# holoskii/Rendering

Hardware: AMD Instinct MI355X
Metric: Mrays/s + ms/frame at 4096^2, 250k-tri BVH scene (higher is better)
Workload: dtype f32

## Files before the change

### include/rtx_debug.h

```cpp
#ifndef RTX_DEBUG_H
#define RTX_DEBUG_H
#include "rtx.h"
#ifdef __cplusplus
extern "C" {
#endif

int rtx_frame_mode(rtx_scene* scene, int* mode, float* split_ms, float* fused_ms);
int rtx_set_frame_mode(rtx_scene* scene, int mode);

int rtx_mesh_flatten_probe(const rtx_mesh* mesh, uint32_t* n_wide, void* wide_out, void* prune_out, uint32_t cap_wide, float* root_rec8);
int rtx_wide_node_slots(void);

int rtx_source_p_probe(const float* tris9, uint32_t n, const double* S3, double sigma, int cam, float* out);

int rtx_cost_grid_read(rtx_scene* scene, uint32_t* out, size_t n, uint32_t* grid_w, uint32_t* grid_h);

int rtx_set_knob(rtx_scene* scene, const char* name, double value);

#define RTX_VARIANT_BOXES    1u
#define RTX_VARIANT_PLAIN    2u
#define RTX_VARIANT_ANALYTIC 4u
#define RTX_VARIANT_STATS    8u
#define RTX_VARIANT_CULL     16u
int rtx_kernel_variant(rtx_scene* scene, uint32_t* bits);

int rtx_ssaa_list_read(rtx_scene* scene, uint32_t* info, uint32_t* scan, size_t n);

int rtx_kernel_time_reset(rtx_scene* scene);
int rtx_kernel_time_stats(rtx_scene* scene, int which, uint32_t* launches, double* total_ms);

int rtx_tile_cost_read(rtx_scene* scene, uint32_t* out, size_t n);

int rtx_math_probe(int device, int op, uint32_t n, const float* x, const float* y, float* out);

int rtx_vec_probe(int device, int op, uint32_t n, const float* a, const float* b, float ior, float* out);

int rtx_desc_serialize(const rtx_scene_desc* desc, void* out, size_t cap, size_t* need);

int rtx_bvh_build_mode(int mode);
int rtx_bvh_launches(const rtx_bvh* bvh, uint32_t* launches, int* queued);

int rtx_scene_mesh_read(rtx_scene* scene, uint32_t mesh, uint32_t* counts2, float* node_bounds, int32_t* node_skip, int32_t* leaf_begin,
                        int32_t* leaf_count, uint32_t* refs);
int rtx_scene_mesh_flat_read(rtx_scene* scene, uint32_t mesh, uint32_t* n_wide, void* wide_out, void* prune_out, uint32_t cap_wide, float* root_rec8);
int rtx_scene_edit_times(rtx_scene* scene, float* ms4);

int rtx_live_device_memory(size_t* allocations, size_t* bytes);

#ifdef __cplusplus
}
#endif
#endif
```

### rendering_amd/__init__.py

```python
import ctypes as C
import os

import numpy as np

HERE = os.path.dirname(os.path.abspath(__file__))
ROOT = os.path.dirname(HERE)
LIB_RTX = os.path.join(HERE, "librtx_hip.so")
LIB_HOST = os.path.join(HERE, "librendering_host.so")

__all__ = ["load", "Scene", "Comm", "RtxError", "device_count", "math_probe", "gather_plan", "exported_symbols"]


class RtxError(RuntimeError):
    pass


class Counters(C.Structure):
    _fields_ = [("rays", C.c_uint64), ("box_tests", C.c_uint64), ("tri_tests", C.c_uint64), ("moot_rays", C.c_uint64)]


_rtx = None
_host = None

RTX_SYMBOLS = [
    "rtx_last_error", "rtx_device_count", "rtx_scene_create", "rtx_scene_destroy", "rtx_scene_set_view", "rtx_scene_bytes",
    "rtx_render_pass1", "rtx_sobel", "rtx_render_ssaa", "rtx_render_frame", "rtx_render_ac", "rtx_frame_status", "rtx_frame_mode", "rtx_set_frame_mode", "rtx_set_knob", "rtx_cost_grid_read", "rtx_mesh_flatten_probe", "rtx_wide_node_slots", "rtx_source_p_probe", "rtx_quantize_bgr8", "rtx_render_frame_host",
    "rtx_counters_enable", "rtx_counters_reset", "rtx_counters_read", "rtx_last_kernel_ms", "rtx_math_probe",
    "rtx_cast_rays", "rtx_trace_rays", "rtx_kernel_time_reset", "rtx_kernel_time_stats", "rtx_tile_cost_read", "rtx_set_row_ownership",
    "rtx_bvh_build", "rtx_bvh_info", "rtx_bvh_read", "rtx_bvh_destroy",
    "rtx_vec_probe", "rtx_desc_serialize", "rtx_bvh_build_mode", "rtx_bvh_launches", "rtx_comm_unique_id", "rtx_comm_create", "rtx_comm_info", "rtx_comm_destroy", "rtx_comm_agree", "rtx_gather", "rtx_gather_plan",
    "rtx_scene_mesh_read", "rtx_scene_mesh_flat_read", "rtx_scene_edit_times", "rtx_kernel_variant", "rtx_ssaa_list_read", "rtx_live_device_memory",
]

RTX_EDIT_SYMBOLS = ["rtx_scene_set_object", "rtx_scene_update_mesh"]

RTX_QUERY_SYMBOLS = ["rtx_occluded_rays"]


def load():
    global _rtx, _host
    if _rtx is not None:
        return _rtx, _host
    for p in (LIB_RTX, LIB_HOST):
        if not os.path.exists(p):
            raise RtxError("native library %s is missing -- build it with ./build.sh (hipcc, gfx950); "
                           "there is no CPU fallback" % p)
    try:
        import torch
    except Exception:
        pass
    rtx = C.CDLL(LIB_RTX, mode=C.RTLD_GLOBAL)
    host = C.CDLL(LIB_HOST, mode=C.RTLD_GLOBAL)
    rtx.rtx_last_error.restype = C.c_char_p
    vp, u32, i32 = C.c_void_p, C.c_uint32, C.c_int
    rtx.rtx_device_count.argtypes = [C.POINTER(C.c_int)]
    rtx.rtx_render_pass1.argtypes = [vp, u32, u32, vp, vp]
    rtx.rtx_sobel.argtypes = [vp, vp, u32, u32, vp, vp]
    rtx.rtx_render_ssaa.argtypes = [vp, vp, u32, u32, vp, vp]
    rtx.rtx_render_frame.argtypes = [vp, u32, u32, vp, vp, vp]
    rtx.rtx_render_ac.argtypes = [vp, vp, vp, vp]
    rtx.rtx_frame_status.argtypes = [vp, C.POINTER(C.c_uint32)]
    rtx.rtx_set_frame_mode.argtypes = [vp, C.c_int]
    rtx.rtx_set_knob.argtypes = [vp, C.c_char_p, C.c_double]
    rtx.rtx_cost_grid_read.argtypes = [vp, vp, C.c_size_t, C.POINTER(C.c_uint32), C.POINTER(C.c_uint32)]
# ... 38 lines not shown
    host.rah_last_error.restype = C.c_char_p
    host.rah_scene_load.restype = vp
    host.rah_scene_load.argtypes = [C.c_char_p, C.c_char_p, i32, i32]
    host.rah_scene_free.argtypes = [vp]
    host.rah_scene_dims.argtypes = [vp] + [C.POINTER(C.c_int)] * 4
    host.rah_scene_resize.argtypes = [vp, i32, i32]
    host.rah_scene_set_device.argtypes = [vp, i32]
    host.rah_set_flag.argtypes = [vp, C.c_char_p, i32]
    host.rah_flatten.restype = vp
    host.rah_flatten.argtypes = [vp]
    host.rah_flat_desc.restype = vp
    host.rah_flat_desc.argtypes = [vp]
    host.rah_flat_free.argtypes = [vp]
    host.rah_bvh_counts.argtypes = [vp, i32, vp]
    host.rah_scene_gpu.restype = vp
    host.rah_scene_gpu.argtypes = [vp]
    host.rah_render_host.argtypes = [vp, vp, i32]
    host.rah_save_bmp.argtypes = [vp, vp, C.c_char_p]
    host.rah_bvh_dump.argtypes = [vp, i32, vp, vp, vp, vp, vp]
    host.rah_tris.argtypes = [vp, i32, vp]
    host.rah_camera.argtypes = [vp, vp, vp, vp, vp]
    host.rah_scene_digest.argtypes = [vp, vp, i32]
    host.rah_view_flags.argtypes = [vp]
    host.rah_load_bmp.argtypes = [C.c_char_p, C.POINTER(C.c_int), C.POINTER(C.c_int), vp, i32]
    host.rah_object_move.argtypes = [vp, i32] + [vp] * 5
    host.rah_object_type.argtypes = [vp, i32]
    host.rah_object_move_times.argtypes = [vp, vp]
    rtx.rtx_scene_set_object.argtypes = [vp, C.c_uint32, vp]
    rtx.rtx_scene_update_mesh.argtypes = [vp, C.c_uint32, vp, vp, vp, vp, vp, i32, vp]
    rtx.rtx_scene_mesh_read.argtypes = [vp, C.c_uint32] + [vp] * 6
    rtx.rtx_scene_mesh_flat_read.argtypes = [vp, C.c_uint32, vp, vp, vp, C.c_uint32, vp]
    rtx.rtx_scene_edit_times.argtypes = [vp, vp]
    rtx.rtx_kernel_variant.argtypes = [vp, C.POINTER(C.c_uint32)]
    rtx.rtx_ssaa_list_read.argtypes = [vp, vp, vp, C.c_size_t]
    rtx.rtx_live_device_memory.argtypes = [C.POINTER(C.c_size_t), C.POINTER(C.c_size_t)]
    _rtx, _host = rtx, host
    return rtx, host


def exported_symbols():
    rtx, _ = load()
    missing = [s for s in RTX_SYMBOLS + RTX_EDIT_SYMBOLS + RTX_QUERY_SYMBOLS if not hasattr(rtx, s)]
    return list(RTX_SYMBOLS), missing


VARIANT_BITS = {"boxes": 1, "plain": 2, "analytic": 4, "stats": 8, "cull": 16}


def _check(rc, what):
    if rc != 0:
        raise RtxError("%s failed (%d): %s" % (what, rc, _rtx.rtx_last_error().decode(errors="replace")))


def device_count():
    rtx, _ = load()
    n = C.c_int(0)
    _check(rtx.rtx_device_count(C.byref(n)), "rtx_device_count")
    return n.value


def live_device_memory():
    rtx, _ = load()
    n, b = C.c_size_t(0), C.c_size_t(0)
    _check(rtx.rtx_live_device_memory(C.byref(n), C.byref(b)), "rtx_live_device_memory")
    return n.value, b.value

# ... 270 lines not shown
                if torch.cuda.is_available():
                    return C.c_void_p(torch.cuda.current_stream().cuda_stream)
            except Exception:
                pass
            return None
        return C.c_void_p(getattr(stream, "cuda_stream", stream))

    def render_pass1(self, fb, rows=None, stream=None):
        r0, r1 = rows if rows is not None else (0, self.height)
        _check(self.rtx.rtx_render_pass1(self.gpu(), r0, r1, C.c_void_p(fb.data_ptr()), self._stream_ptr(stream)),
               "rtx_render_pass1")

    def sobel(self, fb, mask, rows=None, stream=None):
        r0, r1 = rows if rows is not None else (0, self.height)
        _check(self.rtx.rtx_sobel(self.gpu(), C.c_void_p(fb.data_ptr()), r0, r1, C.c_void_p(mask.data_ptr()),
                                  self._stream_ptr(stream)), "rtx_sobel")

    def render_ssaa(self, mask, fb, rows=None, stream=None):
        r0, r1 = rows if rows is not None else (0, self.height)
        _check(self.rtx.rtx_render_ssaa(self.gpu(), C.c_void_p(mask.data_ptr()), r0, r1, C.c_void_p(fb.data_ptr()),
                                        self._stream_ptr(stream)), "rtx_render_ssaa")

    def render_frame(self, fb, mask, rows=None, stream=None):
        r0, r1 = rows if rows is not None else (0, self.height)
        _check(self.rtx.rtx_render_frame(self.gpu(), r0, r1, C.c_void_p(fb.data_ptr()), C.c_void_p(mask.data_ptr()),
                                         self._stream_ptr(stream)), "rtx_render_frame")

    def render_ac(self, fb, counts=None, stream=None):
        cp = C.c_void_p(counts.data_ptr()) if counts is not None else None
        _check(self.rtx.rtx_render_ac(self.gpu(), C.c_void_p(fb.data_ptr()), cp, self._stream_ptr(stream)), "rtx_render_ac")

    def set_knob(self, name, value):
        _check(self.rtx.rtx_set_knob(self.gpu(), name.encode(), float(value)), "rtx_set_knob")

    def kernel_variant(self):
        b = C.c_uint32(0)
        _check(self.rtx.rtx_kernel_variant(self.gpu(), C.byref(b)), "rtx_kernel_variant")
        return {k: bool(b.value & bit) for k, bit in VARIANT_BITS.items()}

    def ssaa_list(self):
        g = self.gpu()
        info = np.zeros(16, np.uint32)
        _check(self.rtx.rtx_ssaa_list_read(g, _np_ptr(info), None, 0), "rtx_ssaa_list_read")
        d = dict(local=bool(info[0]), flagged=int(info[1]), sparse=bool(info[2]), tiles=int(info[3]), tiles_x=int(info[4]),
                 heavy_ticks=int(info[5]), spread_slots=int(info[6]), very=int(info[7]), spread_px=int(info[8]),
                 split4=int(info[9]), split16=int(info[10]), cost_sum=int(info[11]) | int(info[12]) << 32, frame_waves=int(info[13]), scan=None)
        if d["tiles"]:
            scan = np.zeros(2 * d["tiles"] + 1, np.uint32)
            _check(self.rtx.rtx_ssaa_list_read(g, _np_ptr(info), _np_ptr(scan), scan.size), "rtx_ssaa_list_read")
            d["scan"] = scan
        return d

    def cost_grid(self):
        gw, gh = C.c_uint32(0), C.c_uint32(0)
        _check(self.rtx.rtx_cost_grid_read(self.gpu(), None, 0, C.byref(gw), C.byref(gh)), "rtx_cost_grid_read")
        g = np.zeros((gh.value, gw.value, 2), np.uint32)
        _check(self.rtx.rtx_cost_grid_read(self.gpu(), _np_ptr(g), g.size, C.byref(gw), C.byref(gh)), "rtx_cost_grid_read")
        return g[..., 0], g[..., 1]

    def frame_status(self):
        st = C.c_uint32(0)
        _check(self.rtx.rtx_frame_status(self.gpu(), C.byref(st)), "rtx_frame_status")
        return st.value

    def set_frame_mode(self, mode):
        _check(self.rtx.rtx_set_frame_mode(self.gpu(), int(mode)), "rtx_set_frame_mode")
# ... 179 lines not shown
```

### rendering_amd/csrc/rtx_api.hip

```cpp
#include <hip/hip_runtime.h>

#include <cstdio>
#include <dlfcn.h>
#include <algorithm>
#include <array>
#include <functional>
#include <cmath>
#include <cstring>
#include <memory>
#include <string>
#include <type_traits>
#include <vector>

#include "../../include/rtx.h"
#include "../../include/rtx_debug.h"
#include "../../include/rtx_scene_edit.h"
#include "../../include/rtx_query.h"
#include "rtx_device.h"
#include "rtx_own.h"

using namespace rtxd;
using rtxown::DevArray; using rtxown::DevBag; using rtxown::Event; using rtxown::PinnedArray;

#include "rtx_kernels.hip"
#include "rtx_source.hip"
#include "rtx_rays.hip"

hipError_t rtxSortRayKeys(void* temp, size_t* tempBytes, const uint32_t* keysIn, uint32_t* keysOut, uint32_t* order, uint32_t n, int endBit,
                          hipStream_t st);

namespace {

thread_local std::string gErr;

struct RoctxApi { int (*push)(const char*) = nullptr; int (*pop)() = nullptr; };
const RoctxApi& roctx()
{
	static const RoctxApi api = [] {
		RoctxApi a;
		if (!getenv("ROCP_TOOL_LIBRARIES") && !getenv("RTX_ROCTX")) return a;
		void* h = dlopen("librocprofiler-sdk-roctx.so.1", RTLD_NOW | RTLD_GLOBAL);
		if (!h) h = dlopen("libroctx64.so.4", RTLD_NOW | RTLD_GLOBAL);
		if (!h) return a;
		a.push = (int (*)(const char*))dlsym(h, "roctxRangePushA");
		a.pop = (int (*)())dlsym(h, "roctxRangePop");
		if (!a.push || !a.pop) a = RoctxApi();
		return a;
	}();
	return api;
}
struct RoctxRange {
	bool on;
	explicit RoctxRange(const char* name) : on(roctx().push != nullptr) { if (on) roctx().push(name); }
	~RoctxRange() { if (on) roctx().pop(); }
};

int scanExclusive(uint32_t* data, uint32_t n, uint32_t* tmp, hipStream_t st, uint32_t& launches);

int fail(int code, const std::string& msg) { gErr = msg; return code; }
// ... 20 lines not shown
{
	const uint32_t t = m.refs[ref];
	const float* p = m.tri_pos + (size_t)t * 9;
	a.v0x = p[0]; a.v0y = p[1]; a.v0z = p[2]; a.tri = t;
	b.e1x = p[3] - p[0]; b.e1y = p[4] - p[1]; b.e1z = p[5] - p[2];
	b.e2x = p[6] - p[0]; c.e2y = p[7] - p[1]; c.e2z = p[8] - p[2];
}

}

struct Knobs {
	int pass1BlocksPerCU = 0, ssaaBlocksPerCU = 0, frameBlocksPerCU = 0;
	bool prune = true;
	bool sources = true;
	int pruneBoxes = -1;
	bool estimate = true;
	bool estimateShadows = true;
	float costPerRef = 2.0f, costPerLeaf = 95.0f, costBase = 6100.0f;
	float fatFactor = 3.0f;
	uint32_t stripLimit = 100000u;
	uint32_t heavyTicks = 18000u;
	uint32_t spreadSlots = 1u << 20;
	uint32_t splitPercent = 100;
	long long localBelow = -1;
	long long sparseBelow = -1;
	int frameMode = -1;
	uint32_t frameRuleTiles = 65536u, frameRuleTilesAnalytic = 8192u;
	uint32_t frameQueueCap = 0;
	bool debugItems = false;
	int traceReorder = -1;
	int traceOriginFirst = 1;
	int occludedSceneOrder = 0;
	uint32_t dbgTile = 0;
};

struct rtx_scene {
	int device = 0;
	int numCUs = 0;
	Knobs knobs;
	DevBag owned;
	std::vector<Mesh> meshRecs;
	std::vector<DevBag> meshOwned;
	std::vector<Object> objectRecs;
	std::vector<rtx_object> objectDescs;
	DevArray<float> sphereLeafDev;
	DevArray<char> flatScratch;
	float editMs[4] = { 0, 0, 0, 0 };
	Params params;
	bool stats = false;
	bool analytic = true;
	bool boxPrune = false;
	bool plain = true;
	DevArray<float> frames; size_t framesArea = 0;
	DevArray<uint32_t> tileCost, items; size_t tileCap = 0;
	DevArray<uint32_t> ssaaPixels;
	DevArray<uint32_t> work;
	DevArray<unsigned long long> counters;
	DevArray<uint32_t> orderWork;
	int blocksPass1 = 0, blocksSsaa = 0, blocksFrame = 0;
	DevArray<uint32_t> tileDeps; DevArray<unsigned long long> tileFlags; DevArray<uint8_t> tileClass;
	DevArray<unsigned long long> ssaaQueue;
	DevArray<unsigned long long> frameCtl;
	uint32_t epoch = 0;
	std::vector<float> meshBounds;
	struct TileQueues {
		std::vector<uint32_t> key;
		uint32_t* list = nullptr;
		uint8_t* need = nullptr; uint32_t listed = 0;
		uint32_t* countExpect = nullptr; bool needValid = false;
		bool costValid = false;
		uint64_t lastUse = 0;
		float frameMs[2] = { -1.f, -1.f };
		uint32_t frameSamples[2] = { 0, 0 };
		uint32_t framesSeen = 0, generation = 0;
		bool fusedGaveUp = false;
		hipStream_t builtOn = nullptr; Event builtEv;
		void forget()
		{
			key.clear(); costValid = false;
			frameMs[0] = frameMs[1] = -1.f; frameSamples[0] = frameSamples[1] = 0; framesSeen = 0; generation++; fusedGaveUp = false;
		}
	};
	struct LastFused { bool valid = false; uint32_t rowBegin = 0, rowEnd = 0; float* fb = nullptr; uint8_t* mask = nullptr; void* stream = nullptr; size_t queue = ~(size_t)0; uint32_t generation = 0;
	                   uint64_t viewSerial = 0; uint32_t bandH = 0, nParts = 0, part = 0, halo = 0; };
	LastFused lastFused;
	uint32_t framesRecovered = 0;
	DevArray<uint32_t> acCounts, acMax;
	DevArray<uint32_t> rayKeys, rayOrder; size_t rayCap = 0;
// ... 36 lines not shown
	size_t lastFrameQueue = ~(size_t)0;
	std::vector<TileQueues> tileQueues;
	uint64_t tileUse = 0;
	std::vector<Event> evPool[5];
	size_t evUsed[5] = { 0, 0, 0, 0, 0 };
	bool evCollect = false;
};

namespace {

void readKnobs(Knobs& k)
{
	const char* allow = ::getenv("RTX_ALLOW_ENV_KNOBS");
	if (!(allow && allow[0] == '1')) return;
	auto getenv = [](const char* name) { return ::getenv(name); };
	auto num = [](const char* name, long long dflt) { const char* e = ::getenv(name); return e ? strtoll(e, nullptr, 10) : dflt; };
	k.pass1BlocksPerCU = (int)num("RTX_PASS1_BLOCKS_PER_CU", 0); k.ssaaBlocksPerCU = (int)num("RTX_SSAA_BLOCKS_PER_CU", 0); k.frameBlocksPerCU = (int)num("RTX_FRAME_BLOCKS_PER_CU", 0);
	k.prune = !getenv("RTX_NO_PRUNE");
	k.sources = !getenv("RTX_NO_SRC");
	k.pruneBoxes = (int)num("RTX_PRUNE_BOXES", -1);
	k.estimate = !getenv("RTX_NO_COST_ESTIMATE");
	k.estimateShadows = !getenv("RTX_NO_SHADOW_ESTIMATE");
	if (const char* e = getenv("RTX_COST_COEFFS")) sscanf(e, "%f,%f,%f", &k.costPerRef, &k.costPerLeaf, &k.costBase);
	if (const char* e = getenv("RTX_FAT_FACTOR")) k.fatFactor = strtof(e, nullptr);
	k.stripLimit = (uint32_t)num("RTX_STRIP_LIMIT", k.stripLimit);
	k.heavyTicks = (uint32_t)num("RTX_SSAA_HEAVY_TICKS", k.heavyTicks);
	k.spreadSlots = (uint32_t)std::min<long long>(num("RTX_SSAA_SPREAD_SLOTS", k.spreadSlots), 1ll << 20);
	k.splitPercent = (uint32_t)num("RTX_SPLIT_PERCENT", k.splitPercent);
	k.localBelow = num("RTX_SSAA_LOCAL_BELOW", -1);
	k.sparseBelow = num("RTX_SSAA_SPARSE_BELOW", -1);
	if (const char* e = getenv("RTX_FRAME_MODE")) k.frameMode = !strcmp(e, "split") ? 0 : (!strcmp(e, "fused") ? 1 : -1);
	k.frameQueueCap = (uint32_t)num("RTX_FRAME_QUEUE_CAP", 0);
	k.debugItems = getenv("RTX_DEBUG_ITEMS") != nullptr;
	if (const char* e = getenv("RTX_DBG_TILE")) { unsigned tx = 0, ty = 0; if (sscanf(e, "%u,%u", &tx, &ty) == 2) k.dbgTile = ((ty << 16) | tx) + 1; }
}

void chooseBoxPrune(rtx_scene* s)
{
	s->boxPrune = false;
	for (const Object& d : s->objectRecs) {
		if (d.type != RTX_OBJ_MESH) continue;
		if (d.pruneBoxes && s->knobs.pruneBoxes != 0) s->boxPrune = true;
		if (s->knobs.pruneBoxes > 0 && d.prune) s->boxPrune = true;
	}
}

int setView(rtx_scene* s, const rtx_view* v)
{
	if (v->width < 2 || v->height < 2) return fail(RTX_ERR_ARG, "view: width/height must be >= 2");
	View& d = s->params.view;
	d.width = v->width; d.height = v->height; d.bias = v->bias; d.maxDepth = v->max_ray_depth;
	memcpy(d.bg, v->background, 12);
	d.flags = v->flags;
	memcpy(d.camPos, v->cam_pos, 12);
	memcpy(d.camM, v->cam_matrix, 64);
	d.scale = v->scale; d.aspect = v->aspect;
	if ((d.flags & RTX_FLAG_SKYBOX) && !s->params.sky) return fail(RTX_ERR_ARG, "view: skybox flag without skybox faces");
	if (d.maxDepth < 0) d.maxDepth = -1;
	return RTX_OK;
}

constexpr size_t kMaxTimedLaunches = 4096;
constexpr uint32_t kSsaaSpreadSlots = 1u << 20;
constexpr size_t kFrameCtlBytes = 256 * 64;

struct Variant { bool analytic, stats, boxes, cull, plain; };
// ... 33 lines not shown
}
typedef void (*OccludedKernel)(const Params, const uint32_t*, const float*, uint8_t*);
OccludedKernel rayOccludedKernel(const Variant& v, bool sceneOrder)
{
	if (v.analytic) return rtxRayOccludedKernel<false, true, -1, true>;
	return dispatchVariant(v.boxes, v.cull, sceneOrder, [](auto b, auto c, auto ord) -> OccludedKernel { return rtxRayOccludedKernel<true, decltype(b)::value, decltype(c)::value, decltype(ord)::value>; });
}

int askBlocksPerCU(int& perCU, const void* kernel)
{
	if (perCU == 0) { HIPCHK(hipOccupancyMaxActiveBlocksPerMultiprocessor(&perCU, kernel, 256, 0)); perCU = std::max(perCU, 1); }
	return RTX_OK;
}

int residentBlocks(const rtx_scene* s, FrameKernel kernel, int knobPerCU, int* blocks)
{
	int b = 0;
	const int rc = askBlocksPerCU(b, (const void*)kernel);
	if (rc) return rc;
	if (knobPerCU >= 1 && knobPerCU < b) b = knobPerCU;
	*blocks = b * s->numCUs;
	return RTX_OK;
}

int ensureWork(rtx_scene* s)
{
	HIPCHK(hipSetDevice(s->device));
	if (!s->work) {
		HIPCHK(s->work.reserve(256));
		HIPCHK(hipMemset(s->work, 0, 256 * sizeof(uint32_t)));
		HIPCHK(s->orderWork.reserve(8 * 32 * 32));
		HIPCHK(s->counters.reserve(16));
		HIPCHK(hipMemset(s->counters, 0, 16 * sizeof(unsigned long long)));
		Variant v = { false, false, true, true, s->plain };
		int rc;
		if ((rc = residentBlocks(s, pass1Kernel(v), s->knobs.pass1BlocksPerCU, &s->blocksPass1))) return rc;
		v.plain = false;
		if ((rc = residentBlocks(s, ssaaKernel(v), s->knobs.ssaaBlocksPerCU, &s->blocksSsaa))) return rc;
		v.analytic = s->analytic;
		if ((rc = residentBlocks(s, frameKernel(v), s->knobs.frameBlocksPerCU, &s->blocksFrame))) return rc;
	}
	const int blocks = std::max(s->blocksFrame, s->blocksPass1 > s->blocksSsaa ? s->blocksPass1 : s->blocksSsaa);
	const uint32_t totalLanes = (uint32_t)blocks * 256u;
	const int slots = s->params.view.maxDepth + 2;
	const size_t area = (size_t)(slots < 1 ? 1 : slots) * kFrameFields * sizeof(float) * totalLanes;
	const size_t need = 2 * area;
	s->framesArea = area / sizeof(float);
	HIPCHK(s->frames.reserve(need / sizeof(float)));
	const uint32_t txFull = (s->params.view.width + 7) / 8, tyFull = (s->params.view.height + 7) / 8;
	const size_t tiles = (size_t)txFull * tyFull;
	if (tiles > s->tileCap) {
		s->tileCap = 0;
		HIPCHK(s->tileCost.reserve(2 * tiles));
		HIPCHK(s->items.reserve(tiles * 2 + 1 + tiles / 256 + 1024));
		HIPCHK(hipMemset(s->tileCost, 0, 2 * tiles * sizeof(uint32_t)));
		s->tileCap = tiles;
	}
	const size_t pixels = tiles * 64 + kSsaaSpreadSlots;
	HIPCHK(s->ssaaPixels.reserve(pixels));
	s->params.tileCost = s->tileCost;
	s->params.tilesXFull = txFull;
	s->params.frames = s->frames;
	s->params.totalLanes = totalLanes;
	s->params.workCounter = s->work;
	s->params.counters = s->counters;
	return RTX_OK;
}

int prepareView(rtx_scene* s);

int prepBegin(rtx_scene* s)
{
	for (auto& rs : s->renderStreams) {
		if (!rs.active) continue;
		HIPCHK(rs.done.create(hipEventDisableTiming));
		if (hipEventRecord(rs.done, rs.st) == hipSuccess) HIPCHK(hipStreamWaitEvent(nullptr, rs.done, 0));
		else (void)hipGetLastError();
		rs.active = false;
	}
	return RTX_OK;
}
int prepEnd(rtx_scene* s)
{
	HIPCHK(s->evPrepDone.create(hipEventDisableTiming));
	HIPCHK(hipEventRecord(s->evPrepDone, nullptr));
	s->prepRecorded = true; s->prepSeenBy = nullptr;
	for (auto& rs : s->renderStreams) rs.prepSeen = false;
	return RTX_OK;
// ... 27 lines not shown
	const uint32_t nLights = std::min<uint32_t>((uint32_t)s->srcLightPos.size(), kMaxSrcLights);
	bool failed = false;
	for (const auto& sm : s->srcMeshes) {
		if (!sm.base) continue;
		auto build = [&](uint32_t copy, const float* S, double sigma, bool cam) {
			PruneBlock* dst = sm.base + (size_t)copy * sm.nWide;
			if (hipMemcpyAsync(dst, sm.base, (size_t)sm.nWide * sizeof(PruneBlock), hipMemcpyDeviceToDevice, nullptr) != hipSuccess) { failed = true; return; }
			if (!(sigma >= 0.0) || !std::isfinite(sigma) || !std::isfinite((double)S[0] + S[1] + S[2])) return;
			hipLaunchKernelGGL(rtxsrc::rtxSourceRefKernel, dim3((sm.nRefs + 255) / 256), dim3(256), 0, nullptr, sm.refA, sm.refB, sm.refC, sm.nRefs,
			                   (double)S[0], (double)S[1], (double)S[2], sigma, cam ? 1 : 0, sm.refP, sm.blockP);
			hipLaunchKernelGGL(rtxsrc::rtxSourceSlotKernel, dim3(sm.nWide * (kWideSlots / 4)), dim3(256), 0, nullptr, sm.slotRange, sm.nWide, (const float*)sm.refP, (const float*)sm.blockP, dst);
		};
		if (!camSame) build(1, v.camPos, 0.0, true);
		if (!lightsSame)
			for (uint32_t l = 0; l < nLights; l++) {
				if (!s->srcLightIsPoint[l]) continue;
				const float* lp = s->srcLightPos[l].data();
				const double nb = (double)s->srcNmax * std::fabs((double)v.bias);
				const double lpm = std::max(std::fabs((double)lp[0]), std::max(std::fabs((double)lp[1]), std::fabs((double)lp[2])));
				const double sigma = nb * 1.001 + 4.0 * 0x1p-24 * (3.01 * ((double)sm.vmax + kSrcAinfMax + nb) + 2.01 * lpm);
				build(2 + l, lp, sigma, false);
			}
	}
	HIPCHK(hipGetLastError());
	if (failed) { s->srcCamBuilt = false; s->srcLightsBuilt = false; return fail(RTX_ERR_DEVICE, "buildSources: a source copy of the prune records could not be reset"); }
	memcpy(s->srcBuiltCam, v.camPos, 12); s->srcCamBuilt = true;
	s->srcBuiltBias = v.bias; s->srcLightsBuilt = true;
	return RTX_OK;
}

int estimateCosts(rtx_scene* s)
{
	s->costsUsable = false;
	if (!s->knobs.estimate || s->meshLeaves.empty() || !s->tileCost) return RTX_OK;
	const View& v = s->params.view;
	const uint32_t txFull = (v.width + 7) / 8, tyFull = (v.height + 7) / 8;
	const uint32_t gridW = (txFull + 1) / 2, gridH = (tyFull + 1) / 2;
	const size_t cells = (size_t)gridW * gridH;
	HIPCHK(s->costGrid.reserve(2 * cells));
	HIPCHK(hipMemsetAsync(s->costGrid, 0, 2 * cells * sizeof(uint32_t), nullptr));
	SplatSources src;
	memset(&src, 0, sizeof(src));
	if (s->knobs.estimateShadows)
		for (size_t l = 0; l < s->estLights.size() && l < 8; l++)
			for (size_t q = 0; q < s->estPlanes.size() && q < 4 && src.n < 16; q++) {
				const auto& L = s->estLights[l]; const auto& P = s->estPlanes[q];
				src.kind[src.n] = L[3] > 2.5f ? 2 : (int32_t)L[3]; src.weight[src.n] = L[3] > 2.5f ? (uint32_t)((L[3] - 2.0f) / 4.0f) : 1u;
				memcpy(src.l[src.n], L.data(), 12); memcpy(src.p[src.n], P.data(), 24);
				src.n++;
			}
	for (const auto& m : s->meshLeaves)
		if (m.n) hipLaunchKernelGGL(rtxCostSplatKernel, dim3((m.n + 255) / 256, 1 + src.n), dim3(256), 0, nullptr, m.boxes, m.n, v, gridW, gridH, s->costGrid, src);
	const uint32_t tiles = txFull * tyFull;
	FarPlanes far;
	memset(&far, 0, sizeof(far));
	if (s->knobs.estimateShadows) {
		for (size_t q = 0; q < s->estPlanes.size() && q < 4; q++) memcpy(far.p[far.n++], s->estPlanes[q].data(), 24);
		far.farDist = 1500.0f; far.farTicks = 200000u;
	}
	hipLaunchKernelGGL(rtxCostFillKernel, dim3((tiles + 255) / 256), dim3(256), 0, nullptr, (const uint32_t*)s->costGrid, gridW, txFull, tyFull, s->tileCost,
	                   s->knobs.costPerRef, s->knobs.costPerLeaf, s->knobs.costBase, v, far);
	HIPCHK(hipGetLastError());
	s->costsUsable = true;
	return RTX_OK;
}

// ... 734 lines not shown
	if (rc) return rc;
	hipStream_t st = (hipStream_t)stream;
	if (int ro = renderOn(s, st)) return ro;
	if (showNormals(s)) return normalsPass1(s, rowBegin, rowEnd, fb_dev, st);
	Params p = s->params;
	p.fb = fb_dev;
	p.rowBegin = rowBegin; p.rowEnd = rowEnd;
	p.tilesX = (W - 1 + 7) / 8;
	p.tileRow0 = rowBegin / 8;
	const uint32_t lastRow = (rowEnd < H - 1 ? rowEnd : H - 1);
	if (lastRow <= rowBegin) return RTX_OK;
	const uint32_t tilesY = (lastRow + 7) / 8 - p.tileRow0;
	p.nTiles = p.tilesX * tilesY;
	p.tilesY = tilesY;
#if RTX_DBG
	p.pad3 = s->knobs.dbgTile;
#endif
	p.workCounter = s->work + 128;
	if (p.view.width > 0x7fff8u || p.view.height > 0x7fff8u) return fail(RTX_ERR_ARG, "frame too large");
	rtx_scene::TileQueues* tq = nullptr;
	if ((rc = buildTileList(s, rowBegin, lastRow, p.tilesX, p.tileRow0, tilesY, &tq, true, st))) return rc;
	p.tileList = tq->list;
	p.stripBit = stripsFit(p.view) ? 0x10000000u : 0u;
	if (tq->costValid || s->costsUsable) {
		const uint32_t stripLimit = s->knobs.stripLimit;
		const unsigned pieces = tq->listed > 16384u ? 32u : 1u;
		if (pieces > 1) hipLaunchKernelGGL(rtxTileOrderKernel<false>, dim3(pieces, 8), dim3(256), 0, st, s->orderWork, tq->list, s->tileCost, s->params.tilesXFull, s->orderedList, (const uint8_t*)nullptr,
		                   (const unsigned long long*)nullptr, 1u, 0u, 0u, (uint32_t*)nullptr, p.tilesX, stripLimit, (uint32_t*)nullptr, p.stripBit);
		hipLaunchKernelGGL(rtxTileOrderKernel<true>, dim3(pieces, 8), dim3(256), 0, st, s->orderWork, tq->list, s->tileCost, s->params.tilesXFull, s->orderedList, (const uint8_t*)nullptr,
		                   (const unsigned long long*)nullptr, 1u, 0u, 0u, (uint32_t*)nullptr, p.tilesX, stripLimit, s->work + 128, p.stripBit);
		p.tileList = s->orderedList;
	}
	else HIPCHK(hipMemsetAsync(s->work + 128, 0, 128 * sizeof(uint32_t), st));
	tq->costValid = true;
	uint32_t blocks = (uint32_t)s->blocksPass1;
	const uint32_t wavesNeeded = (p.nTiles + 3) / 4;
	if (blocks > wavesNeeded) blocks = wavesNeeded ? wavesNeeded : 1;
	if ((rc = stamp(s, 0, st))) return rc;
	hipLaunchKernelGGL(pass1Kernel(variantOf(s)), dim3(blocks), dim3(256), 0, st, p);
	HIPCHK(hipGetLastError());
	if ((rc = stamp(s, 0, st))) return rc;
	return RTX_OK;
}

static int renderFrameFused(rtx_scene* s, uint32_t rowBegin, uint32_t rowEnd, float* fb_dev, uint8_t* mask_dev, void* stream, bool costsKnown)
{
	RoctxRange range("one launch (rtxFrameKernel)");
	const uint32_t W = s->params.view.width, H = s->params.view.height;
	if (rowEnd > H) rowEnd = H;
	if (rowBegin >= rowEnd) return RTX_OK;
	int rc = ensureWork(s);
	if (rc) return rc;
	hipStream_t st = (hipStream_t)stream;
	Params p = s->params;
	p.fb = fb_dev;
	p.maskOut = mask_dev;
	p.rowBegin = rowBegin; p.rowEnd = rowEnd;
	p.tilesX = (W - 1 + 7) / 8;
	p.tileRow0 = rowBegin / 8;
	if (p.view.width > 0xffffu || p.view.height > 0xffffu) return fail(RTX_ERR_ARG, "frame too large");
	const size_t maskBytes = (size_t)(rowEnd - rowBegin) * W;
	const bool maskInClear = maskBytes <= (4u << 20);
	const uint32_t lastRow = (rowEnd < H - 1 ? rowEnd : H - 1);
	if (!maskInClear || lastRow <= rowBegin) HIPCHK(hipMemsetAsync(mask_dev + (size_t)rowBegin * W, 0, maskBytes, st));
	if (lastRow <= rowBegin) return RTX_OK;
	const uint32_t tilesY = (lastRow + 7) / 8 - p.tileRow0;
	p.nTiles = p.tilesX * tilesY;
	p.tilesY = tilesY;
	p.tilesYFull = (H + 7) / 8;
	p.workCounter = s->work + 128;
	rtx_scene::TileQueues* tq = nullptr;
// ... 146 lines not shown
	else { s->lastFused.valid = false; rc = renderFrameSplit(s, rowBegin, rowEnd, fb_dev, mask_dev, stream); }
	if (rc) { if (s->evUsed[3] & 1) s->evUsed[3]--; return rc; }
	if ((rc = stamp(s, 3, st))) return rc;
	if (pr) {
		HIPCHK(hipEventRecord(pr->b, st));
		pr->mode = warm ? mode : -1; pr->queue = (size_t)(tq - s->tileQueues.data()); pr->generation = tq->generation; pr->pending = true; pr->refresh = reprobe;
	}
	if (tq) tq->framesSeen++;
	if (tq) tq->costValid = true;
	s->lastFrameMode = mode;
	s->lastFrameQueue = tq ? (size_t)(tq - s->tileQueues.data()) : ~(size_t)0;
	return RTX_OK;
}

int rtx_set_knob(rtx_scene* s, const char* name, double value)
{
	if (!s || !name) return fail(RTX_ERR_ARG, "scene/name is NULL");
	Knobs& k = s->knobs;
	const std::string n = name;
	if (n == "strip_limit") k.stripLimit = (uint32_t)value;
	else if (n == "ssaa_heavy_ticks") k.heavyTicks = (uint32_t)value;
	else if (n == "ssaa_spread_slots") k.spreadSlots = (uint32_t)std::min(value, (double)kSsaaSpreadSlots);
	else if (n == "split_percent") k.splitPercent = (uint32_t)value;
	else if (n == "ssaa_local_below") k.localBelow = (long long)value;
	else if (n == "ssaa_sparse_below") k.sparseBelow = (long long)value;
	else if (n == "frame_queue_cap") k.frameQueueCap = (uint32_t)value;
	else if (n == "verify_lists") s->verifyLists = value != 0;
	else if (n == "frame_rule_tiles") k.frameRuleTiles = value >= 4294967295.0 ? 0xffffffffu : (uint32_t)value;
	else if (n == "frame_rule_tiles_analytic") k.frameRuleTilesAnalytic = value >= 4294967295.0 ? 0xffffffffu : (uint32_t)value;
	else if (n == "debug_items") k.debugItems = value != 0;
	else if (n == "trace_reorder") k.traceReorder = value < 0 ? -1 : (value != 0 ? 1 : 0);
	else if (n == "trace_key_origin_first") k.traceOriginFirst = value != 0 ? 1 : 0;
	else if (n == "occluded_scene_order") k.occludedSceneOrder = value != 0 ? 1 : 0;
	else if (n == "prune_boxes") {
		k.pruneBoxes = value < 0 ? -1 : (value != 0 ? 1 : 0);
		chooseBoxPrune(s);
		s->rayHitBlocks[0] = s->rayHitBlocks[1] = 0;
		for (auto& b : s->rayOccludedBlocks) b[0] = b[1] = 0;
	}
	else return fail(RTX_ERR_ARG, "unknown knob: " + n);
	return RTX_OK;
}

int rtx_kernel_variant(rtx_scene* s, uint32_t* bits)
{
	if (!s || !bits) return fail(RTX_ERR_ARG, "scene/bits is NULL");
	const Variant v = variantOf(s);
	*bits = (v.boxes ? RTX_VARIANT_BOXES : 0u) | (v.plain ? RTX_VARIANT_PLAIN : 0u) | (v.analytic ? RTX_VARIANT_ANALYTIC : 0u) |
	        (v.stats ? RTX_VARIANT_STATS : 0u) | (v.cull ? RTX_VARIANT_CULL : 0u);
	return RTX_OK;
}

int rtx_ssaa_list_read(rtx_scene* s, uint32_t* info, uint32_t* scan, size_t n)
{
	if (!s || !info) return fail(RTX_ERR_ARG, "scene/info is NULL");
	HIPCHK(hipSetDevice(s->device));
	HIPCHK(hipDeviceSynchronize());
	memset(info, 0, 16 * sizeof(uint32_t));
	uint32_t w[20] = { 0 };
	if (s->work) HIPCHK(hipMemcpy(w, s->work, sizeof(w), hipMemcpyDeviceToHost));
	info[0] = w[8]; info[1] = w[9]; info[2] = w[11];
	info[3] = s->ssaaListTiles; info[4] = s->params.tilesXFull; info[5] = s->ssaaListHeavy; info[6] = s->ssaaListSpread;
	info[7] = RTX_SSAA_VERY; info[8] = RTX_SSAA_SPREAD_PX;
	info[9] = w[18]; info[10] = w[19]; info[11] = w[16]; info[12] = w[17];
	info[13] = (uint32_t)s->blocksFrame * 4u;
	if (!scan) return RTX_OK;
	if (!s->ssaaListTiles || !s->items) return fail(RTX_ERR_ARG, "no SSAA list has been built");
	if (n != 2 * (size_t)s->ssaaListTiles + 1) return fail(RTX_ERR_ARG, "n must be 2 tiles + 1 of the last list");
	HIPCHK(hipMemcpy(scan, s->items, n * sizeof(uint32_t), hipMemcpyDeviceToHost));
	return RTX_OK;
}

int rtx_set_frame_mode(rtx_scene* s, int mode)
// ... 608 lines not shown
```

Measured before the change: 17620.

## Add flat-tile prepass that renders simple diffuse tiles before pass1

Adds a kernel that runs before pass1. It renders cheap tiles, meaning tiles outside the mesh rectangle and under a cost threshold with only primitive hits, diffuse materials and point or directional lights. It uses a specialized wave-uniform tracer with no recursion and no BVH. Rendered tiles are marked done in the ordered tile list, so pass1 skips them, and per-tile flags remember which tiles succeeded or bailed for later frames. This is meant to cut the general kernel's overhead on trivial tiles. The cost is an extra launch, a possible list copy, and wasted work on tiles that bail.

```diff
diff --git a/include/rtx_debug.h b/include/rtx_debug.h
--- a/include/rtx_debug.h
+++ b/include/rtx_debug.h
@@ -23,6 +23,8 @@
 #define RTX_VARIANT_STATS    8u
 #define RTX_VARIANT_CULL     16u
 int rtx_kernel_variant(rtx_scene* scene, uint32_t* bits);
+
+int rtx_flat_tiles_read(rtx_scene* scene, uint32_t* out3);
 
 int rtx_ssaa_list_read(rtx_scene* scene, uint32_t* info, uint32_t* scan, size_t n);
 
diff --git a/rendering_amd/__init__.py b/rendering_amd/__init__.py
--- a/rendering_amd/__init__.py
+++ b/rendering_amd/__init__.py
@@ -29,7 +29,7 @@
     "rtx_cast_rays", "rtx_trace_rays", "rtx_kernel_time_reset", "rtx_kernel_time_stats", "rtx_tile_cost_read", "rtx_set_row_ownership",
     "rtx_bvh_build", "rtx_bvh_info", "rtx_bvh_read", "rtx_bvh_destroy",
     "rtx_vec_probe", "rtx_desc_serialize", "rtx_bvh_build_mode", "rtx_bvh_launches", "rtx_comm_unique_id", "rtx_comm_create", "rtx_comm_info", "rtx_comm_destroy", "rtx_comm_agree", "rtx_gather", "rtx_gather_plan",
-    "rtx_scene_mesh_read", "rtx_scene_mesh_flat_read", "rtx_scene_edit_times", "rtx_kernel_variant", "rtx_ssaa_list_read", "rtx_live_device_memory",
+    "rtx_scene_mesh_read", "rtx_scene_mesh_flat_read", "rtx_scene_edit_times", "rtx_kernel_variant", "rtx_ssaa_list_read", "rtx_live_device_memory", "rtx_flat_tiles_read",
 ]
 
 RTX_EDIT_SYMBOLS = ["rtx_scene_set_object", "rtx_scene_update_mesh"]
@@ -134,6 +134,8 @@
     rtx.rtx_scene_mesh_flat_read.argtypes = [vp, C.c_uint32, vp, vp, vp, C.c_uint32, vp]
     rtx.rtx_scene_edit_times.argtypes = [vp, vp]
     rtx.rtx_kernel_variant.argtypes = [vp, C.POINTER(C.c_uint32)]
+    if hasattr(rtx, "rtx_flat_tiles_read"):
+        rtx.rtx_flat_tiles_read.argtypes = [vp, vp]
     rtx.rtx_ssaa_list_read.argtypes = [vp, vp, vp, C.c_size_t]
     rtx.rtx_live_device_memory.argtypes = [C.POINTER(C.c_size_t), C.POINTER(C.c_size_t)]
     _rtx, _host = rtx, host
@@ -470,6 +472,11 @@
 
     def set_knob(self, name, value):
         _check(self.rtx.rtx_set_knob(self.gpu(), name.encode(), float(value)), "rtx_set_knob")
+
+    def flat_tiles(self):
+        out = np.zeros(3, np.uint32)
+        _check(self.rtx.rtx_flat_tiles_read(self.gpu(), _np_ptr(out)), "rtx_flat_tiles_read")
+        return int(out[0]), int(out[1]), int(out[2])
 
     def kernel_variant(self):
         b = C.c_uint32(0)
diff --git a/rendering_amd/csrc/rtx_api.hip b/rendering_amd/csrc/rtx_api.hip
--- a/rendering_amd/csrc/rtx_api.hip
+++ b/rendering_amd/csrc/rtx_api.hip
@@ -25,6 +25,7 @@
 #include "rtx_kernels.hip"
 #include "rtx_source.hip"
 #include "rtx_rays.hip"
+#include "rtx_flat.hip"
 
 hipError_t rtxSortRayKeys(void* temp, size_t* tempBytes, const uint32_t* keysIn, uint32_t* keysOut, uint32_t* order, uint32_t n, int endBit,
                           hipStream_t st);
@@ -111,6 +112,7 @@
 	int traceOriginFirst = 1;
 	int occludedSceneOrder = 0;
 	uint32_t dbgTile = 0;
+	int flatTiles = 1;
 };
 
 struct rtx_scene {
@@ -133,6 +135,7 @@
 	DevArray<float> frames; size_t framesArea = 0;
 	DevArray<uint32_t> tileCost, items; size_t tileCap = 0;
 	DevArray<uint32_t> ssaaPixels;
+	DevArray<uint8_t> flatFlag; DevArray<uint32_t> flatCounts; uint32_t flatSet = 0; bool flatLaunched = false;
 	DevArray<uint32_t> work;
 	DevArray<unsigned long long> counters;
 	DevArray<uint32_t> orderWork;
@@ -235,6 +238,7 @@
 	if (const char* e = getenv("RTX_FRAME_MODE")) k.frameMode = !strcmp(e, "split") ? 0 : (!strcmp(e, "fused") ? 1 : -1);
 	k.frameQueueCap = (uint32_t)num("RTX_FRAME_QUEUE_CAP", 0);
 	k.debugItems = getenv("RTX_DEBUG_ITEMS") != nullptr;
+	k.flatTiles = (int)num("RTX_FLAT_TILES", k.flatTiles);
 	if (const char* e = getenv("RTX_DBG_TILE")) { unsigned tx = 0, ty = 0; if (sscanf(e, "%u,%u", &tx, &ty) == 2) k.dbgTile = ((ty << 16) | tx) + 1; }
 }
 
@@ -334,6 +338,8 @@
 		HIPCHK(s->orderWork.reserve(8 * 32 * 32));
 		HIPCHK(s->counters.reserve(16));
 		HIPCHK(hipMemset(s->counters, 0, 16 * sizeof(unsigned long long)));
+		HIPCHK(s->flatCounts.reserve(8));
+		HIPCHK(hipMemset(s->flatCounts, 0, 8 * sizeof(uint32_t)));
 		Variant v = { false, false, true, true, s->plain };
 		int rc;
 		if ((rc = residentBlocks(s, pass1Kernel(v), s->knobs.pass1BlocksPerCU, &s->blocksPass1))) return rc;
@@ -356,6 +362,8 @@
 		HIPCHK(s->tileCost.reserve(2 * tiles));
 		HIPCHK(s->items.reserve(tiles * 2 + 1 + tiles / 256 + 1024));
 		HIPCHK(hipMemset(s->tileCost, 0, 2 * tiles * sizeof(uint32_t)));
+		HIPCHK(s->flatFlag.reserve(tiles));
+		HIPCHK(hipMemset(s->flatFlag, 0, tiles));
 		s->tileCap = tiles;
 	}
 	const size_t pixels = tiles * 64 + kSsaaSpreadSlots;
@@ -449,6 +457,7 @@
 int estimateCosts(rtx_scene* s)
 {
 	s->costsUsable = false;
+	if (s->flatFlag && s->tileCap) HIPCHK(hipMemsetAsync(s->flatFlag, 0, s->tileCap, nullptr));
 	if (!s->knobs.estimate || s->meshLeaves.empty() || !s->tileCost) return RTX_OK;
 	const View& v = s->params.view;
 	const uint32_t txFull = (v.width + 7) / 8, tyFull = (v.height + 7) / 8;
@@ -1249,11 +1258,26 @@
 		p.tileList = s->orderedList;
 	}
 	else HIPCHK(hipMemsetAsync(s->work + 128, 0, 128 * sizeof(uint32_t), st));
+	const int flatMode = (s->stats || RTX_DBG) ? 0 : s->knobs.flatTiles;
+	bool flat = flatMode == 2 || (flatMode == 1 && s->plain && !s->analytic && p.tileList == s->orderedList);
+	if (flat && p.tileList != s->orderedList) {
+		HIPCHK(hipMemcpyAsync(s->orderedList, tq->list, (16 + (size_t)tq->listed) * sizeof(uint32_t), hipMemcpyDeviceToDevice, st));
+		p.tileList = s->orderedList;
+	}
+	s->flatLaunched = flat;
 	tq->costValid = true;
 	uint32_t blocks = (uint32_t)s->blocksPass1;
 	const uint32_t wavesNeeded = (p.nTiles + 3) / 4;
 	if (blocks > wavesNeeded) blocks = wavesNeeded ? wavesNeeded : 1;
 	if ((rc = stamp(s, 0, st))) return rc;
+	if (flat) {
+		const uint32_t flatBlocks = (tq->listed + 4 * kFlatPerWave - 1) / (4 * kFlatPerWave);
+		s->flatSet ^= 1u;
+		FlatRect seen;
+		meshTileRect(s, p.tilesXFull, (p.view.height + 7) / 8, seen.r);
+		hipLaunchKernelGGL(rtxFlatTileKernel, dim3(flatBlocks ? flatBlocks : 1), dim3(256), 0, st, p, s->orderedList.get(), s->flatFlag.get(), s->flatCounts.get(),
+		                   (uint32_t)flatMode, s->flatSet, (p.view.height + 7) / 8, seen);
+	}
 	hipLaunchKernelGGL(pass1Kernel(variantOf(s)), dim3(blocks), dim3(256), 0, st, p);
 	HIPCHK(hipGetLastError());
 	if ((rc = stamp(s, 0, st))) return rc;
@@ -1466,6 +1490,7 @@
 	else if (n == "trace_reorder") k.traceReorder = value < 0 ? -1 : (value != 0 ? 1 : 0);
 	else if (n == "trace_key_origin_first") k.traceOriginFirst = value != 0 ? 1 : 0;
 	else if (n == "occluded_scene_order") k.occludedSceneOrder = value != 0 ? 1 : 0;
+	else if (n == "flat_tiles") k.flatTiles = value >= 2 ? 2 : (value >= 1 ? 1 : 0);
 	else if (n == "prune_boxes") {
 		k.pruneBoxes = value < 0 ? -1 : (value != 0 ? 1 : 0);
 		chooseBoxPrune(s);
@@ -1473,6 +1498,17 @@
 		for (auto& b : s->rayOccludedBlocks) b[0] = b[1] = 0;
 	}
 	else return fail(RTX_ERR_ARG, "unknown knob: " + n);
+	return RTX_OK;
+}
+
+int rtx_flat_tiles_read(rtx_scene* s, uint32_t* out3)
+{
+	if (!s || !out3) return fail(RTX_ERR_ARG, "scene/out is NULL");
+	out3[0] = out3[1] = out3[2] = 0;
+	if (!s->flatLaunched || !s->flatCounts) return RTX_OK;
+	HIPCHK(hipSetDevice(s->device));
+	HIPCHK(hipDeviceSynchronize());
+	HIPCHK(hipMemcpy(out3, s->flatCounts + 3 * s->flatSet, 3 * sizeof(uint32_t), hipMemcpyDeviceToHost));
 	return RTX_OK;
 }
 
diff --git a/rendering_amd/csrc/rtx_flat.hip b/rendering_amd/csrc/rtx_flat.hip
--- /dev/null
+++ b/rendering_amd/csrc/rtx_flat.hip
@@ -0,0 +1,188 @@
+
+namespace {
+
+constexpr uint32_t kFlatDone = 0xffffffffu;
+constexpr uint32_t kFlatPerWave = 16;
+constexpr uint32_t kFlatTryTicks = 4000u;
+struct FlatRect { uint32_t r[4]; };
+
+__device__ __forceinline__ bool flatTrace(const Params& P, bool active, bool shadow, V3 o, V3 d, float tmax, int& hobj, float& ht)
+{
+	hobj = -1; ht = tmax;
+	const float ix = 1 / d.x, iy = 1 / d.y, iz = 1 / d.z;
+	const bool sx = ix < 0, sy = iy < 0, sz = iz < 0;
+	bool live = active;
+	const uint32_t nObj = uni(P.nObjects);
+	for (uint32_t oi = 0; oi < nObj; oi = uni(oi + 1)) {
+		const Object* ob = uni(P.objects + oi);
+		const u32x16 rec = sload16(ob);
+		const int type = (int)rec[0];
+		const int mat = (int)rec[1];
+		const bool consider = live && !(shadow && mat == 2);
+		if (ballot(consider) == 0) continue;
+		if (type == 3) {
+			const u32x16 rec2 = sload16((const char*)ob + 64);
+			const uint32_t mflags = rec2[13];
+			bool pending = consider;
+			if ((mflags & 1u) != 0) {
+				const float xlo = (F(rec2[2]) - o.x) * ix, xhi = (F(rec2[3]) - o.x) * ix, ylo = (F(rec2[4]) - o.y) * iy, yhi = (F(rec2[5]) - o.y) * iy;
+				const float zlo = (F(rec2[6]) - o.z) * iz, zhi = (F(rec2[7]) - o.z) * iz;
+				float tmin = sx ? xhi : xlo, tmx = sx ? xlo : xhi;
+				const float tymin = sy ? yhi : ylo, tymax = sy ? ylo : yhi;
+				bool fail = (tmin > tymax) || (tymin > tmx);
+				if (tymin > tmin) tmin = tymin;
+				if (tymax < tmx) tmx = tymax;
+				const float tzmin = sz ? zhi : zlo, tzmax = sz ? zlo : zhi;
+				fail = fail || (tmin > tzmax) || (tzmin > tmx);
+				pending = consider && !fail;
+			}
+			if (ballot(pending) != 0) return false;
+		}
+		else {
+			const V3 c = mk(F(rec[2]), F(rec[3]), F(rec[4]));
+			float t0 = kFltMax; bool hit;
+			if (type == 1) {
+				const float r2 = F(rec[5]);
+				const V3 L = c - o;
+				const float tca = dot(L, d);
+				const float d2 = dot(L, L) - tca * tca;
+				hit = !(d2 > r2);
+				const float thc = __builtin_sqrtf(r2 - d2);
+				t0 = tca - thc;
+				const float t1 = tca + thc;
+				if (t0 < 0) t0 = t1;
+				if (t0 < 0) hit = false;
+			}
+			else {
+				const V3 n = mk(F(rec[6]), F(rec[7]), F(rec[8]));
+				const float denom = dot(d, n);
+				hit = !(fabsf(denom) < RTX_EPS8);
+				t0 = dot(c - o, n) / denom;
+				hit = hit && (t0 >= 0);
+			}
+			if (consider && hit && t0 < ht) { hobj = (int)oi; ht = t0; }
+		}
+		live = live && !(shadow && hobj >= 0);
+	}
+	return true;
+}
+
+__device__ __forceinline__ bool flatTile(const Params& P, bool valid, V3 o, V3 d, V3& col)
+{
+	col = mk(0, 0, 0);
+	if (0 > P.view.maxDepth) { if (valid) col = skyColor(P, d); return true; }
+	int hobj; float ht;
+	if (!flatTrace(P, valid, false, o, d, kFltMax, hobj, ht)) return false;
+	const bool shaded = valid && hobj >= 0;
+	if (valid && hobj < 0) col = skyColor(P, d);
+	if (ballot(shaded) == 0) return true;
+	const V3 Ph = o + d * ht;
+	V3 N = mk(0, 0, 0), objColor = mk(0, 0, 0);
+	for (uint64_t rem = ballot(shaded); rem != 0;) {
+		const int o0 = __builtin_amdgcn_readlane(hobj, __builtin_ctzll(rem));
+		const Object* ob = uni(P.objects + o0);
+		const u32x16 a = sload16(ob);
+		if ((int)a[1] != 0) return false;
+		const bool mine = shaded && hobj == o0;
+		if (mine) {
+			objColor = mk(F(a[10]), F(a[11]), F(a[12]));
+			if ((int)a[0] == 1) N = normalized(Ph - mk(F(a[2]), F(a[3]), F(a[4])));
+			else N = mk(F(a[6]), F(a[7]), F(a[8]));
+		}
+		rem &= ~ballot(mine);
+	}
+	V3 diff = mk(0, 0, 0);
+	const uint32_t nLights = uni(P.nLights);
+	for (uint32_t li = 0; li < nLights; li = uni(li + 1)) {
+		const u32x16 w = sload16(P.lights + li);
+		const int lt = (int)w[0];
+		if (lt != 1 && lt != 2) return false;
+		const V3 lcol = mk(F(w[1]), F(w[2]), F(w[3]));
+		const float intensity = F(w[4]);
+		V3 L, I; float dist;
+		if (lt == 1) {
+			L = mk(F(w[5]), F(w[6]), F(w[7]));
+			I = lcol * intensity;
+			dist = kFltMax;
+		}
+		else {
+			const V3 lp = mk(F(w[8]), F(w[9]), F(w[10]));
+			V3 Lp = Ph - lp;
+			I = lcol * attenuation(intensity, len2(Lp));
+			L = normalized(Lp);
+			dist = length(Ph - lp);
+		}
+		const V3 nL = -L;
+		const bool moot = fmaxRef(0.f, dot(N, nL)) == 0.f;
+		int sobj; float st;
+		if (!flatTrace(P, shaded && !moot, true, Ph + N * P.view.bias, nL, dist, sobj, st)) return false;
+		const float vis = (sobj < 0) ? 1.0f : 0.0f;
+		const float c = vis * fmaxRef(0.f, dot(N, nL));
+		if (shaded) diff = diff + I * c;
+	}
+	if (shaded) col = objColor * diff;
+	return true;
+}
+
+}
+
+__global__ void __launch_bounds__(256) rtxFlatTileKernel(const Params P, uint32_t* __restrict__ list, uint8_t* __restrict__ flags, uint32_t* __restrict__ counts,
+                                                         uint32_t mode, uint32_t set, uint32_t tilesYFull, const FlatRect seen)
+{
+	const uint32_t lane = __lane_id();
+	const uint32_t wave = uni((blockIdx.x * blockDim.x + threadIdx.x) >> 6), nWaves = gridDim.x * (blockDim.x >> 6);
+	if (blockIdx.x == 0 && threadIdx.x < 3) counts[3 * (set ^ 1u) + threadIdx.x] = 0;
+	const u32x16 head = sload16(list);
+	uint32_t total = 0;
+	for (int q = 0; q < 8; ++q) total += head[8 + q];
+	uint32_t nTried = 0, nBailed = 0, nRendered = 0;
+	for (uint32_t first = 0; first < total; first = uni(first + kFlatPerWave * nWaves)) {
+		uint32_t at = 0, tile = kFlatDone, cell = 0;
+		bool cand = false;
+		const uint32_t g = first + lane * nWaves + wave;
+		if (lane < kFlatPerWave && g < total) {
+			uint32_t r = g;
+			for (int q = 0; q < 8; ++q) {
+				const uint32_t n = head[8 + q];
+				if (at == 0 && r < n) at = head[q] + r;
+				if (at == 0) r -= n;
+			}
+		}
+		if (at != 0) {
+			tile = list[at];
+			const uint32_t tx = tile & 0xffffu, ty = tile >> 16;
+			if (tile != kFlatDone && !(tile & (P.stripBit | 0x8000u)) && tx < P.tilesX && tx < P.tilesXFull && ty < tilesYFull) {
+				cell = ty * P.tilesXFull + tx;
+				const uint32_t f = flags[cell];
+				const bool inSeen = tx >= seen.r[0] && tx < seen.r[1] && ty >= seen.r[2] && ty < seen.r[3];
+				cand = mode == 2u || f == 1u || (f == 0u && !inSeen && P.tileCost[cell] <= kFlatTryTicks);
+			}
+		}
+		for (uint64_t rem = ballot(cand); rem != 0; rem &= rem - 1) {
+			const int src = __builtin_ctzll(rem);
+			const uint32_t t = (uint32_t)__builtin_amdgcn_readlane((int)tile, src), a = (uint32_t)__builtin_amdgcn_readlane((int)at, src);
+			const uint32_t c = (uint32_t)__builtin_amdgcn_readlane((int)cell, src);
+			const uint32_t x = (t & 0xffffu) * 8 + (lane & 7), y = (t >> 16) * 8 + (lane >> 3);
+			const bool valid = x < P.view.width - 1 && y < P.view.height - 1 && y >= P.rowBegin && y < P.rowEnd && rowRendered(P, y);
+			nTried++;
+			if (ballot(valid) == 0) { nRendered++; if (lane == 0) list[a] = kFlatDone; continue; }
+			const unsigned long long t0 = wall_clock64();
+			V3 o, d, col;
+			primaryRay(P, (float)x + 0.5f, (float)y + 0.5f, o, d);
+			const bool done = flatTile(P, valid, o, d, col);
+			if (!done) { nBailed++; if (lane == 0) flags[c] = 2; continue; }
+			nRendered++;
+			if (valid) {
+				float* px = P.fb + ((size_t)y * P.view.width + x) * 3;
+				px[0] = col.x; px[1] = col.y; px[2] = col.z;
+			}
+			const unsigned long long dt = wall_clock64() - t0;
+			if (lane == 0) {
+				P.tileCost[c] = dt > 0xffffffffull ? 0xffffffffu : (uint32_t)dt;
+				flags[c] = 1;
+				list[a] = kFlatDone;
+			}
+		}
+	}
+	if (lane == 0 && nTried) { atomicAdd(counts + 3 * set, nTried); atomicAdd(counts + 3 * set + 1, nBailed); atomicAdd(counts + 3 * set + 2, nRendered); }
+}
```

Result: slower. 15590 (-11.5%).
